# mks0601/ExAvatar_RELEASE

Hardware: AMD Instinct MI355X
Metric: train iters/sec (fwd+bwd raster) at 1024x1024 / ~150k Gaussians (higher is better)
Workload: dtype f32

## Files before the change

### exavatar_release_amd/csrc/blend.h

```cpp
#pragma once
#include "common.h"

namespace exa {

typedef float v2f __attribute__((ext_vector_type(2)));
typedef float v4f __attribute__((ext_vector_type(4)));

struct BatchLds {
    float px[BATCH], py[BATCH], ca[BATCH], cb[BATCH], cc[BATCH], op[BATCH];
    float4 col[BATCH];
};

__device__ __forceinline__ void stage_splat(BatchLds& s, int lane, const float2& r0, const float4& r1, const float4& r2) {
    s.px[lane] = r0.x; s.py[lane] = r0.y;
    s.ca[lane] = r1.x; s.cb[lane] = r1.y; s.cc[lane] = r1.z; s.op[lane] = __builtin_amdgcn_logf(r1.w);
    s.col[lane] = r2;
}

__device__ __forceinline__ bool conic_safe(float ca, float cb, float cc) {
    const float tr = ca + cc;
    return ca <= 0.0f && cc <= 0.0f && 4.0f * ca * cc - cb * cb >= 1e-5f * (tr * tr);
}

struct Alpha2 { v2f alpha, A, Ag, p2; bool vis0, vis1; };
__device__ __forceinline__ Alpha2 splat_alpha2(v2f px, v2f py, v2f ca, v2f cb, v2f cc, v2f lop, float fx, float fy, bool live) {
#pragma clang fp contract(off)
    const v2f dx = px - fx, dy = py - fy;
    const v2f t = __builtin_elementwise_fma(cb, dy, ca * dx);
    const v2f u = __builtin_elementwise_fma(cc * dy, dy, lop);
    Alpha2 r;
    r.p2 = __builtin_elementwise_fma(t, dx, u);
    r.A.x = __builtin_amdgcn_exp2f(r.p2.x);
    r.A.y = __builtin_amdgcn_exp2f(r.p2.y);
    const float a0 = fminf(ALPHA_MAX, r.A.x), a1 = fminf(ALPHA_MAX, r.A.y);
    r.vis0 = a0 >= ALPHA_MIN;
    r.vis1 = a1 >= ALPHA_MIN;
    r.alpha.x = r.vis0 ? a0 : 0.0f;
    r.alpha.y = r.vis1 ? a1 : 0.0f;
    r.Ag.x = (r.vis0 && live) ? r.A.x : 0.0f;
    r.Ag.y = (r.vis1 && live) ? r.A.y : 0.0f;
    return r;
}

struct Ops4 { v4f px, py, ca, cb, cc, op; };
__device__ __forceinline__ Ops4 load_ops4(const BatchLds& s, int k) {
    Ops4 o;
    o.px = *reinterpret_cast<const v4f*>(&s.px[k]);
    o.py = *reinterpret_cast<const v4f*>(&s.py[k]);
    o.ca = *reinterpret_cast<const v4f*>(&s.ca[k]);
    o.cb = *reinterpret_cast<const v4f*>(&s.cb[k]);
    o.cc = *reinterpret_cast<const v4f*>(&s.cc[k]);
    o.op = *reinterpret_cast<const v4f*>(&s.op[k]);
    return o;
}
struct Alpha4 { float alpha[4], Ag[4], p2[4]; unsigned long long took[4]; };
__device__ __forceinline__ Alpha4 splat_alpha4(const Ops4& o, float fx, float fy, bool live) {
    const Alpha2 lo = splat_alpha2(o.px.xy, o.py.xy, o.ca.xy, o.cb.xy, o.cc.xy, o.op.xy, fx, fy, live);
    const Alpha2 hi = splat_alpha2(o.px.zw, o.py.zw, o.ca.zw, o.cb.zw, o.cc.zw, o.op.zw, fx, fy, live);
    Alpha4 r;
    r.alpha[0] = lo.alpha.x; r.alpha[1] = lo.alpha.y; r.alpha[2] = hi.alpha.x; r.alpha[3] = hi.alpha.y;
    r.Ag[0] = lo.Ag.x; r.Ag[1] = lo.Ag.y; r.Ag[2] = hi.Ag.x; r.Ag[3] = hi.Ag.y;
    r.p2[0] = lo.p2.x; r.p2[1] = lo.p2.y; r.p2[2] = hi.p2.x; r.p2[3] = hi.p2.y;
    r.took[0] = __builtin_amdgcn_ballot_w64(lo.vis0); r.took[1] = __builtin_amdgcn_ballot_w64(lo.vis1);
    r.took[2] = __builtin_amdgcn_ballot_w64(hi.vis0); r.took[3] = __builtin_amdgcn_ballot_w64(hi.vis1);
    return r;
}
__device__ __forceinline__ void power_guard4(Alpha4& e, const Ops4& o, uint32_t unsafe4) {
    const float lop[4] = {o.op.x, o.op.y, o.op.z, o.op.w};
#pragma unroll
    for (int j = 0; j < 4; ++j) {
        if ((unsafe4 >> j) & 1u) {
            const bool neg = e.p2[j] <= lop[j];
            e.alpha[j] = neg ? e.alpha[j] : 0.0f;
            e.Ag[j] = neg ? e.Ag[j] : 0.0f;
            e.took[j] &= __builtin_amdgcn_ballot_w64(neg);
        }
    }
}

__device__ __forceinline__ void blend_group4(float& T, float& Tdead, unsigned long long live_mask, const float (&alpha)[4],
                                             float (&Tb)[4], float (&w)[4], float (&gate)[4]) {
#pragma clang fp contract(off)
    Tb[0] = T;
    w[0] = alpha[0] * Tb[0]; Tb[1] = Tb[0] - w[0];
    w[1] = alpha[1] * Tb[1]; Tb[2] = Tb[1] - w[1];
    w[2] = alpha[2] * Tb[2]; Tb[3] = Tb[2] - w[2];
    w[3] = alpha[3] * Tb[3];
    const float T4 = Tb[3] - w[3];
    if ((__builtin_amdgcn_ballot_w64(T4 < T_EPS) & live_mask) != 0ull) {
        const float after[4] = {Tb[1], Tb[2], Tb[3], T4};
        const bool dies = T4 < T_EPS && T > 0.0f;
        float Tn = T;
#pragma unroll
        for (int j = 0; j < 4; ++j) {
            const bool stop = after[j] < T_EPS;
            w[j] = stop ? 0.0f : w[j];
            gate[j] = stop ? 0.0f : gate[j];
            Tn = stop ? Tn : after[j];
        }
        Tdead = dies ? Tn : Tdead;
        T = (T4 < T_EPS) ? 0.0f : T4;
    } else {
        T = T4;
    }
}
__device__ __forceinline__ void blend_group4(float& T, float& Tdead, unsigned long long live_mask, const float (&alpha)[4],
                                             float (&Tb)[4], float (&w)[4]) {
    float none[4] = {0.f, 0.f, 0.f, 0.f};
    blend_group4(T, Tdead, live_mask, alpha, Tb, w, none);
}

}
```

### exavatar_release_amd/csrc/render_bwd.hip

```cpp
#include <stdlib.h>
#include "blend.h"

namespace exa {

constexpr int RBLOCK = 64;
template <int GC> struct XLayout;
template <> struct XLayout<16> {
    static constexpr int ROW = 36, GROUP = 16 * 36, FLOATS = 4 * 16 * 36;
    static constexpr int WK = ROW;
    __device__ static __forceinline__ int g(int lane) { return lane % 16; }
    __device__ static __forceinline__ int h(int lane) { return lane / 16; }
    __device__ static __forceinline__ int wbase(int lane) { return (lane / 16) * GROUP + 2 * (lane % 16); }
    __device__ static __forceinline__ int rbase(int lane) { return h(lane) * GROUP + g(lane) * ROW; }
    __device__ static __forceinline__ float reduce(float x) {
        x += __shfl_xor(x, 16, 64);
        x += __shfl_xor(x, 32, 64);
        return x;
    }
    __device__ static __forceinline__ void reduce9(float& a, float& b, float& c, float& d, float& e, float& f, float& g,
                                                   float& h, float& i) {
        a = reduce(a); b = reduce(b); c = reduce(c); d = reduce(d); e = reduce(e); f = reduce(f); g = reduce(g);
        h = reduce(h); i = reduce(i);
    }
};
// ... 127 lines not shown
            const int sx0 = r3.x & 0xffff, sx1 = r3.x >> 16, sy0 = r3.y & 0xffff;
            p.pslot = r3.w + (uint32_t)((sub.gsy - sy0) * (sx1 - sx0) + (sub.gsx - sx0));
            if (PREFIX && !trainable(h.id)) p.pslot = NO_SLOT;
        }
        const float* cf = a.bw.ckpt + (size_t)(b0 + (n + BATCH - 1) / BATCH) * (5 * 64) + lane;
        const float* cs = a.bw.ckpt + (size_t)slot * (5 * 64) + lane;
        if ((int)slot > b0) { p.cs0 = cs[0]; p.cs1 = cs[64]; p.cs2 = cs[128]; p.cs3 = cs[192]; p.cs4 = HAS_DEPTH ? cs[256] : 0.f; }
        p.cf0 = cf[0]; p.cf1 = cf[64]; p.cf2 = cf[128]; p.cf3 = cf[192]; p.cf4 = HAS_DEPTH ? cf[256] : 0.f;
        const int pxi = sub.ox + (lane & 7), pyi = sub.oy + (lane >> 3);
        if (pxi < a.grid.W && pyi < a.grid.H) {
            const size_t HW = (size_t)a.grid.W * a.grid.H;
            const size_t pix = (size_t)pyi * a.grid.W + pxi;
            p.gr = dL_dcolor[pix];
            p.gg = dL_dcolor[HW + pix];
            p.gb = dL_dcolor[2 * HW + pix];
            if (HAS_DEPTH && a.dL_ddepth) p.gd = a.dL_ddepth[pix];
            if (a.dL_dalpha) p.ga = a.dL_dalpha[pix];
        }
        return p;
    };

    uint32_t first_slot = wg * SPW;
    if (SPW == 1 && gridDim.y == 1) {
        const uint32_t m0 = a.tw.bwd_meta[0], m1 = a.tw.bwd_meta[1], magic = a.tw.bwd_meta[2];
        const uint32_t mapped = a.bw.bucket ? reinterpret_cast<const uint32_t*>(a.bw.bucket)[min(wg, nslots - 1u)] : 0u;
        if (magic == BWD_ORDER_MAGIC && a.bw.bucket) {
            if (wg >= m0 + m1) return;
            first_slot = mapped;
        }
    }
    BwdHdr hh[SPW];
    BwdPay pp[SPW];
#pragma unroll
    for (int i = 0; i < SPW; ++i) hh[i] = load_hdr(first_slot + i);
#pragma unroll
    for (int i = 0; i < SPW; ++i) pp[i] = load_pay(hh[i], first_slot + i);
#pragma unroll
    for (int rep = 0; rep < SPW; ++rep) {
    const BwdHdr& h0 = hh[rep];
    const BwdPay& p0 = pp[rep];
    const uint32_t slot = first_slot + rep;
    if (is_active(h0)) {
    const uint32_t bm_lo = __builtin_amdgcn_readfirstlane(h0.bm_lo), bm_hi = __builtin_amdgcn_readfirstlane(h0.bm_hi);
    const int st = (int)__builtin_amdgcn_readfirstlane(h0.st1) - 1;
    const int b0 = (int)(__builtin_amdgcn_readfirstlane(h0.begin) / BATCH);
    const int bq = (int)slot - b0;
    const int cnt = __popc(bm_lo) + __popc(bm_hi);
    const bool flagged = (((lane < 32 ? bm_lo : bm_hi) >> (lane & 31)) & 1u) != 0u;
    const int below = mask_rank(bm_lo, bm_hi);
    const int dst = flagged ? below : cnt + (lane - below);
    const SubTile sub = decode_subtile(st, a.grid);
    const int pxi = sub.ox + (lane & 7), pyi = sub.oy + (lane >> 3);
    const bool inside = pxi < a.grid.W && pyi < a.grid.H;
    const float fx = (float)pxi, fy = (float)pyi;
    const float gr = p0.gr, gg = p0.gg, gb = p0.gb, gd = p0.gd, ga = p0.ga;

    stage_splat(s_b, dst, p0.r0, p0.r1, p0.r2);
    s_pslot[dst] = p0.pslot;
    s_pg[(lane >> 4) * 17 + (lane & 15)] = make_float4(gr, gg, gb, gd);

    float T = inside ? 1.0f : 0.0f, Tdead = 1.0f;
    float sr = 0.f, sg = 0.f, sb = 0.f, sd = 0.f;
    if (bq > 0) {
        T = fmaxf(p0.cs0, 0.0f);
        sr = p0.cs1; sg = p0.cs2; sb = p0.cs3; sd = p0.cs4;
    }
    const float T_final = p0.cf0;
    const float tail = T_final * (ga - (bg[0] * gr + bg[1] * gg + bg[2] * gb));
    float R = (p0.cf1 - sr) * gr + (p0.cf2 - sg) * gg + (p0.cf3 - sb) * gb - tail;
    if (HAS_DEPTH) R = fmaf(p0.cf4 - sd, gd, R);
    wave_lds_fence();
    const unsigned long long unsafe = __builtin_amdgcn_ballot_w64(!conic_safe(s_b.ca[lane], s_b.cb[lane], s_b.cc[lane]));
    const unsigned long long need = PREFIX ? __ballot(lane < cnt && s_pslot[lane] != NO_SLOT) : ~0ull;

    const int g = XL::g(lane), h = XL::h(lane);
    float2* const xw_row = reinterpret_cast<float2*>(s_x + XL::wbase(lane));
    const float4* const xr_row = reinterpret_cast<const float4*>(s_x + XL::rbase(lane));

    for (int c0 = 0; c0 < cnt; c0 += GC) {
        if (__all(T == 0.0f)) break;
        const int cend = min(cnt, c0 + GC);
        {
            auto grad4 = [&](Alpha4& e, unsigned long long live_mask, const float4 (&col)[4], int k) {
                float Tb[4], w[4];
                blend_group4(T, Tdead, live_mask, e.alpha, Tb, w, e.Ag);
                float2* x = xw_row + (k - c0) * (XL::WK / 2);
#pragma unroll
                for (int u = 0; u < 4; ++u) {
                    const float4 c = col[u];
                    float cg = fmaf(c.z, gb, fmaf(c.y, gg, c.x * gr));
                    if (HAS_DEPTH) cg = fmaf(c.w, gd, cg);
                    R = fmaf(-cg, w[u], R);
                    const float inv = __builtin_amdgcn_rcpf(1.0f - e.alpha[u]);
                    const float dLda = fmaf(Tb[u], cg, -(R * inv));
                    x[u * (XL::WK / 2)] = make_float2(e.Ag[u] * dLda, w[u]);
                }
            };
            auto group4 = [&](const Ops4& ops, int k) {
                float4 col[4] = {s_b.col[k], s_b.col[k + 1], s_b.col[k + 2], s_b.col[k + 3]};
                if (!HAS_DEPTH) { keep_b128(col[0]); keep_b128(col[1]); keep_b128(col[2]); keep_b128(col[3]); }
                const bool live = T > 0.0f;
                const unsigned long long live_mask = __builtin_amdgcn_ballot_w64(live);
                Alpha4 e = splat_alpha4(ops, fx, fy, live);
                if ((unsafe >> k) & 0xfull) power_guard4(e, ops, (uint32_t)((unsafe >> k) & 0xfull));
                grad4(e, live_mask, col, k);
            };
            Ops4 opsA = load_ops4(s_b, c0);
            for (int k = c0; k < cend; k += 8) {
                const Ops4 opsB = load_ops4(s_b, (k + 4) & 63);
                group4(opsA, k);
                if (k + 4 >= cend) break;
                opsA = load_ops4(s_b, (k + 8) & 63);
                group4(opsB, k + 4);
            }
        }
        wave_lds_fence();
        if (!PREFIX || ((need >> c0) & ((1ull << GC) - 1ull)) != 0ull) {
            const int kk = c0 + g;
            float S0 = 0.f, Sx = 0.f, Sxx = 0.f, Sy = 0.f, Sxy = 0.f, dr = 0.f, dg = 0.f, db = 0.f, dz = 0.f;
#pragma unroll
            for (int j = 0; j < GC / 2; ++j) {
                const float4 v = xr_row[j];
#pragma unroll
                for (int t = 0; t < 2; ++t) {
                    const int q = 2 * j + t;
                    const float aG = t ? v.z : v.x, wq = t ? v.w : v.y;
                    const int pp = h * GC + q;
                    float4 pg = s_pg[(pp >> 4) * 17 + (pp & 15)];
                    if (!HAS_DEPTH) keep_b128(pg);
                    const float X = (float)((q & 7) - 4);
                    S0 += aG;
                    if ((q & 7) != 4) { Sx = fmaf(aG, X, Sx); Sxx = fmaf(aG, X * X, Sxx); }
                    if (q >> 3) {
                        Sy += aG;
                        if ((q & 7) != 4) Sxy = fmaf(aG, X, Sxy);
                    }
                    dr = fmaf(wq, pg.x, dr); dg = fmaf(wq, pg.y, dg); db = fmaf(wq, pg.z, db);
                    if (HAS_DEPTH) dz = fmaf(wq, pg.w, dz);
                }
            }
            const float u0 = s_b.px[kk] - (float)(sub.ox + 4), v0 = s_b.py[kk] - (float)(sub.oy + (GC / 8) * h);
            float mx = fmaf(u0, S0, -Sx), my = fmaf(v0, S0, -Sy);
            float mxx = fmaf(u0, mx - Sx, Sxx);
            float mxy = fmaf(v0, mx, fmaf(-u0, Sy, Sxy));
            float myy = fmaf(v0, my - Sy, Sy);
            float dop = S0;
            XL::reduce9(mx, my, mxx, mxy, myy, dop, dr, dg, db);
            if (HAS_DEPTH) dz = XL::reduce(dz);
            if (h == 0 && kk < cend) {
                const float inv_o = __builtin_amdgcn_exp2f(-s_b.op[kk]);
                const uint32_t ps = s_pslot[kk];
                if (!PREFIX || ps != NO_SLOT) {
                    char* dst = partial_at(prec, ps);
                    *reinterpret_cast<partial_v4*>(dst) = partial_v4{mx, my, mxx, mxy};
                    *reinterpret_cast<partial_v4*>(dst + 16) = partial_v4{myy, dop * inv_o, dr, dg};
                    if (PARTIAL_BYTES == 40) *reinterpret_cast<partial_v2*>(dst + 32) = partial_v2{db, dz};
                    else *reinterpret_cast<partial_v4*>(dst + 32) = partial_v4{db, dz, 0.f, 0.f};
                    if (PARTIAL_BYTES == 64) *reinterpret_cast<partial_v4*>(dst + 48) = partial_v4{0.f, 0.f, 0.f, 0.f};
                    touched[ps] = (uint8_t)1;
                }
            }
        }
        wave_lds_fence();
    }
    }
    }
}

hipError_t launch_render_bwd(const RenderBwdArgs* a, int K, hipStream_t s) {
    uint64_t slots = 0;
    bool depth = false, prefix = false;
    for (int k = 0; k < K; ++k) {
        uint64_t mine = a[k].capacity / BATCH;
        if (a[k].used_slots && a[k].used_slots < mine) mine = a[k].used_slots;
        slots = mine > slots ? mine : slots;
        depth = depth || a[k].dL_ddepth != nullptr;
        prefix = prefix || a[k].grad_first > 0;
    }
    if (slots == 0) return hipSuccess;
#ifndef EXA_BWD_GC
#define EXA_BWD_GC 8
#endif
#ifndef EXA_BWD_SPW
#define EXA_BWD_SPW 1
#endif
#ifndef EXA_BWD_WPB
#define EXA_BWD_WPB 1
#endif
#ifndef EXA_BWD_LDS_PAD
#define EXA_BWD_LDS_PAD 0
#endif
    constexpr int GC = EXA_BWD_GC, SPW = EXA_BWD_SPW, WPB = EXA_BWD_WPB;
    const Batch<RenderBwdArgs> b = make_batch(a, K);
    const dim3 grid((unsigned)((slots + SPW * WPB - 1) / (SPW * WPB)), K);
    if (prefix) {
        const dim3 g1((unsigned)((slots + WPB - 1) / WPB), K);
        if (depth) render_bwd_kernel<true, GC, 1, true, WPB><<<g1, RBLOCK * WPB, (size_t)EXA_BWD_LDS_PAD, s>>>(b);
        else render_bwd_kernel<false, GC, 1, true, WPB><<<g1, RBLOCK * WPB, (size_t)EXA_BWD_LDS_PAD, s>>>(b);
    } else if (depth) {
        render_bwd_kernel<true, GC, SPW, false, WPB><<<grid, RBLOCK * WPB, (size_t)EXA_BWD_LDS_PAD, s>>>(b);
    } else {
        render_bwd_kernel<false, GC, SPW, false, WPB><<<grid, RBLOCK * WPB, (size_t)EXA_BWD_LDS_PAD, s>>>(b);
    }
// ... 5 lines not shown
```

### exavatar_release_amd/csrc/render_fwd.hip

```cpp
#include <stdlib.h>
#include "blend.h"

namespace exa {

constexpr int RBLOCK = 64;

constexpr int SORT_TILE = 2048;
constexpr int SBLOCK = 256;

template <int E>
__device__ __forceinline__ void lds_merge_sort(const unsigned long long* gkeys, int n, uint32_t* __restrict__ sorted,
                                               unsigned long long* keys_out, unsigned long long* buf, int tid) {
    constexpr int NPAD = SBLOCK * E;
    const int lane = tid & 63;
    unsigned long long key[E];
#pragma unroll
    for (int e = 0; e < E; ++e) {
        const int i = e * SBLOCK + tid;
        key[e] = i < n ? gkeys[i] : ~0ull;
        buf[i] = key[e];
    }
    __syncthreads();
    {
        uint32_t rank[E];
// ... 389 lines not shown
        static_assert(ORDER_LDS_WORDS <= SORT_TILE, "order_slots borrows the bucket counters of the sort");
        order_slots(a.tw, a.store_ctx ? reinterpret_cast<uint32_t*>(a.bw.bucket) : nullptr, a.grid.subtiles, (int)blockIdx.x, tid,
                    s_cnt, [&](int st) { return a.tw.ranges[st]; });
        return;
    }
#ifdef EXA_PROBE_SORT
    const unsigned long long t0 = __builtin_readcyclecounter();
#endif
    if (blockIdx.x == ORDER_WGS && tid == 0 && (uint64_t)a.tw.header->num_rendered > a.capacity) a.tw.header->overflow = 1u;
    const int wg = (int)blockIdx.x - ORDER_WGS;
    if (wg >= (int)a.tw.header->active_cells * SUBS_PER_CELL) return;
    if (SPLIT && a.tw.cell_long[wg >> 6] == 0u) return;
    const int st = (int)a.tw.cell_desc[wg >> 6].x * SUBS_PER_CELL + (wg & 63);
    const uint2 range = a.tw.ranges[st];
    const int n = (int)(range.y - range.x);
    if (n == 0) return;
    unsigned long long* gkeys = a.bw.keys + range.x;
    uint32_t* sorted = a.bw.sorted + range.x;
    unsigned long long* const keys_out = KEEP ? gkeys : nullptr;
    if (n <= 64) {
        if (!SPLIT && tid < 64) wave_rank_sort64(gkeys, n, sorted, keys_out, s_buf, tid);
        return;
    }
    if (n > SORT_TILE) {
        for (int first = 0; first < n; first += 8 * SBLOCK) rank_sort_list<8>(gkeys, n, first, sorted, s_buf, tid);
        if (keys_out) {
            __threadfence_block();
            __syncthreads();
            for (int i = tid; i < n; i += SBLOCK) {
                const uint32_t id = sorted[i];
                keys_out[i] = ((unsigned long long)__float_as_uint(a.splats[id].depth) << 32) | id;
            }
        }
        return;
    }
    bool done;
    if (n <= 256) done = lds_bucket_sort<1>(gkeys, n, sorted, keys_out, s_buf, s_cnt, s_misc, tid);
    else if (n <= 512) done = lds_bucket_sort<2>(gkeys, n, sorted, keys_out, s_buf, s_cnt, s_misc, tid);
    else if (n <= 1024) done = lds_bucket_sort<4>(gkeys, n, sorted, keys_out, s_buf, s_cnt, s_misc, tid);
    else done = lds_bucket_sort<8>(gkeys, n, sorted, keys_out, s_buf, s_cnt, s_misc, tid);
    if (done) return;
    __syncthreads();
    if (n <= 256) lds_merge_sort<1>(gkeys, n, sorted, keys_out, s_buf, tid);
    else if (n <= 512) lds_merge_sort<2>(gkeys, n, sorted, keys_out, s_buf, tid);
    else if (n <= 1024) lds_merge_sort<4>(gkeys, n, sorted, keys_out, s_buf, tid);
    else lds_merge_sort<8>(gkeys, n, sorted, keys_out, s_buf, tid);
#ifdef EXA_PROBE_SORT
    __syncthreads();
    if (tid == 0) a.tw.part_cnt[st] = (uint32_t)(__builtin_readcyclecounter() - t0);
#endif
}

template <bool STORE, bool TWO>
__global__ __launch_bounds__(RBLOCK) void render_fwd_kernel(Batch<RenderFwdArgs> batch) {
    __shared__ BatchLds s_b;

    const RenderFwdArgs& a = batch.v[blockIdx.y];
    if ((int)blockIdx.x >= a.grid.subtiles) return;
    const int lane = threadIdx.x;
#ifdef EXA_PROBE_FWD
    const unsigned long long t0 = wall_clock64();
#endif
    const uint4 slot = a.tw.slots[blockIdx.x];
    const SubTile sub = decode_subtile((int)slot.z, a.grid);
    const int st = sub.st;
    if (sub.ox >= a.grid.W || sub.oy >= a.grid.H) return;
    const int pxi = sub.ox + (lane & 7), pyi = sub.oy + (lane >> 3);
    const bool inside = pxi < a.grid.W && pyi < a.grid.H;
    const float fx = (float)pxi, fy = (float)pyi;
    const uint2 range = TWO ? a.tw.ranges[slot.z] : make_uint2(slot.x, slot.y);
    const int n = (int)(range.y - range.x);
    if (TWO && n == 0 && reuse_a_pixels(a.src_color, a.src_bg, a.bg)) {
        if (inside) {
            const size_t HW = (size_t)a.grid.W * a.grid.H, pix = (size_t)pyi * a.grid.W + pxi;
            const float c0 = a.src_color[pix], c1 = a.src_color[HW + pix], c2 = a.src_color[2 * HW + pix];
            const float d = a.src_depth[pix], al = a.src_alpha[pix];
            a.out_color[pix] = c0; a.out_color[HW + pix] = c1; a.out_color[2 * HW + pix] = c2;
            a.out_depth[pix] = d; a.out_alpha[pix] = al;
        }
        if (STORE && lane == 0) a.tw.fwd_exit[st] = make_uint2(0u, 0u);
        return;
    }

    float T = inside ? 1.0f : 0.0f, Tdead = 1.0f;
    v2f Crg = {0.f, 0.f}, Cbd = {0.f, 0.f};
    const Splat* __restrict__ splats = a.splats;
    const uint32_t* __restrict__ sorted = a.bw.sorted + range.x;
    auto record = [&](uint32_t id) -> const float4* {
        if (TWO) return reinterpret_cast<const float4*>(((id & SRC_B) ? a.splats2 : splats) + (id & ~SRC_B));
        return reinterpret_cast<const float4*>(splats + id);
    };

    uint32_t id_next = 0;
    float2 r0 = make_float2(0.f, 0.f);
    float4 r1 = make_float4(0.f, 0.f, 0.f, 0.f), r2 = r1;
    if (n > 0) {
        const uint32_t id0 = lane < n ? sorted[lane] : 0u;
        if (64 + lane < n) id_next = sorted[64 + lane];
        if (lane < n) {
            const float4* rec = record(id0);
            r0 = *reinterpret_cast<const float2*>(rec); r1 = rec[1]; r2 = rec[2];
        }
    }
    float* ckpt = a.bw.ckpt + (size_t)(range.x / BATCH) * (5 * 64) + lane;
    int entered = 0;
    for (int base = 0; base < n; base += 64) {
        if (__all(T == 0.0f)) break;
        if (STORE && base > 0) {
            float* c = ckpt + (size_t)entered * (5 * 64);
            c[0] = T > 0.0f ? T : -Tdead; c[64] = Crg.x; c[128] = Crg.y; c[192] = Cbd.x; c[256] = Cbd.y;
        }
        ++entered;
        const unsigned long long unsafe = __builtin_amdgcn_ballot_w64(!conic_safe(r1.x, r1.y, r1.z));
        stage_splat(s_b, lane, r0, r1, r2);
        {
            const int jn = base + 64 + lane;
            r0 = make_float2(0.f, 0.f); r1 = make_float4(0.f, 0.f, 0.f, 0.f); r2 = r1;
            if (jn < n) {
                const float4* rec = record(id_next);
                r0 = *reinterpret_cast<const float2*>(rec); r1 = rec[1]; r2 = rec[2];
            }
            if (jn + 64 < n) id_next = sorted[jn + 64];
        }
        wave_lds_fence();
        const int cnt = min(64, n - base);
        unsigned long long blended = 0ull;
        auto blend4 = [&](const Alpha4& e, const float4& c0, const float4& c1, const float4& c2, const float4& c3, int k) -> bool {
#ifdef EXA_FWD_SKIP_VOTE
            const float amax = fmaxf(fmaxf(e.alpha[0], e.alpha[1]), fmaxf(e.alpha[2], e.alpha[3])) * T;
            if (!__any(amax > 0.0f)) return false;
#endif
            const unsigned long long live_mask = __builtin_amdgcn_ballot_w64(T > 0.0f);
            if (STORE) {
                auto vote_bit = [&](int j, uint32_t bit) -> uint32_t {
                    const unsigned long long m = e.took[j] & live_mask;
                    uint32_t r;
                    asm("s_cmp_lg_u64 %1, 0\n\ts_cselect_b32 %0, %2, 0" : "=s"(r) : "s"(m), "s"(bit) : "scc");
                    return r;
                };
                const uint32_t nib = vote_bit(0, 1u) | vote_bit(1, 2u) | vote_bit(2, 4u) | vote_bit(3, 8u);
                blended |= (unsigned long long)nib << k;
            }
            float Tb[4], w[4];
            blend_group4(T, Tdead, live_mask, e.alpha, Tb, w);
            Crg = __builtin_elementwise_fma(v2f{c0.x, c0.y}, v2f{w[0], w[0]}, Crg);
            Cbd = __builtin_elementwise_fma(v2f{c0.z, c0.w}, v2f{w[0], w[0]}, Cbd);
            Crg = __builtin_elementwise_fma(v2f{c1.x, c1.y}, v2f{w[1], w[1]}, Crg);
            Cbd = __builtin_elementwise_fma(v2f{c1.z, c1.w}, v2f{w[1], w[1]}, Cbd);
            Crg = __builtin_elementwise_fma(v2f{c2.x, c2.y}, v2f{w[2], w[2]}, Crg);
            Cbd = __builtin_elementwise_fma(v2f{c2.z, c2.w}, v2f{w[2], w[2]}, Cbd);
            Crg = __builtin_elementwise_fma(v2f{c3.x, c3.y}, v2f{w[3], w[3]}, Crg);
            Cbd = __builtin_elementwise_fma(v2f{c3.z, c3.w}, v2f{w[3], w[3]}, Cbd);
#ifdef EXA_FWD_EXIT4
            return __all(T == 0.0f);
#else
            return (k & 4) ? __all(T == 0.0f) : false;
#endif
        };
        auto group4 = [&](const Ops4& ops, int k) -> bool {
            const float4 c0 = s_b.col[k], c1 = s_b.col[k + 1], c2 = s_b.col[k + 2], c3 = s_b.col[k + 3];
            Alpha4 e = splat_alpha4(ops, fx, fy, true);
            if ((unsafe >> k) & 0xfull) power_guard4(e, ops, (uint32_t)((unsafe >> k) & 0xfull));
            return blend4(e, c0, c1, c2, c3, k);
        };
        Ops4 opsA = load_ops4(s_b, 0);
        for (int k = 0; k < cnt; k += 8) {
            const Ops4 opsB = load_ops4(s_b, (k + 4) & 63);
            if (group4(opsA, k)) break;
            if (k + 4 >= cnt) break;
            opsA = load_ops4(s_b, (k + 8) & 63);
            if (group4(opsB, k + 4)) break;
        }
        if (STORE && lane == 0) a.bw.bmask[range.x / BATCH + (uint32_t)(entered - 1)] = blended;
        wave_lds_fence();
    }

    const size_t HW = (size_t)a.grid.W * a.grid.H;
    if (inside) {
        const size_t pix = (size_t)pyi * a.grid.W + pxi;
        const float* __restrict__ bg = a.bg;
        const float Tf = T > 0.0f ? T : Tdead;
        a.out_color[pix] = Crg.x + Tf * bg[0];
        a.out_color[HW + pix] = Crg.y + Tf * bg[1];
        a.out_color[2 * HW + pix] = Cbd.x + Tf * bg[2];
        a.out_depth[pix] = Cbd.y;
        a.out_alpha[pix] = 1.0f - Tf;
    }
    if (STORE) {
        if (lane == 0) a.tw.fwd_exit[st] = make_uint2((uint32_t)n, (uint32_t)entered);
#ifdef EXA_PROBE_FWD
        if (lane == 0) {
            a.tw.part_cnt[4 * blockIdx.x] = (uint32_t)t0;
            a.tw.part_cnt[4 * blockIdx.x + 1] = (uint32_t)wall_clock64();
            const uint32_t hw = __builtin_amdgcn_s_getreg((31 << 11) | 4), xcc = __builtin_amdgcn_s_getreg((31 << 11) | 20);
            a.tw.part_cnt[4 * blockIdx.x + 2] = (hw & 0xffffu) | ((xcc & 0xfu) << 16);
        }
#endif
        if (n > 0) {
            float* c = ckpt + (size_t)((n + BATCH - 1) / BATCH) * (5 * 64);
            c[0] = T > 0.0f ? T : Tdead; c[64] = Crg.x; c[128] = Crg.y; c[192] = Cbd.x; c[256] = Cbd.y;
        }
    }
}

static int max_subtiles(const RenderFwdArgs* a, int K) {
    int n = 0;
    for (int k = 0; k < K; ++k) n = max(n, a[k].grid.subtiles);
    return n;
}

hipError_t launch_sort_subtiles(const RenderFwdArgs* a, int K, hipStream_t s) {
    const int subtiles = max_subtiles(a, K);
    if (subtiles == 0) return hipSuccess;
    const int split_at = dev_knobs().split_subtiles;
    bool keep = false;
    for (int k = 0; k < K; ++k) keep = keep || a[k].keep_sorted_keys != 0;
    const dim3 grid(subtiles + ORDER_WGS, K);
    if (subtiles >= split_at) {
        sort_short_kernel<<<dim3((subtiles + SBLOCK / 64 - 1) / (SBLOCK / 64), K), SBLOCK, 0, s>>>(make_batch(a, K));
        if (keep) sort_subtiles_kernel<true, true><<<grid, SBLOCK, 0, s>>>(make_batch(a, K));
        else sort_subtiles_kernel<true, false><<<grid, SBLOCK, 0, s>>>(make_batch(a, K));
    } else {
        if (keep) sort_subtiles_kernel<false, true><<<grid, SBLOCK, 0, s>>>(make_batch(a, K));
        else sort_subtiles_kernel<false, false><<<grid, SBLOCK, 0, s>>>(make_batch(a, K));
    }
    return hipGetLastError();
}

#ifndef EXA_FWD_LDS_PAD
#define EXA_FWD_LDS_PAD 0
#endif
hipError_t launch_render_fwd(const RenderFwdArgs* a, int K, hipStream_t s) {
    const int subtiles = max_subtiles(a, K);
    if (subtiles == 0) return hipSuccess;
    constexpr int pad = EXA_FWD_LDS_PAD;
    if (a[0].splats2) {
        if (a[0].store_ctx) render_fwd_kernel<true, true><<<dim3(subtiles, K), RBLOCK, (size_t)pad, s>>>(make_batch(a, K));
        else render_fwd_kernel<false, true><<<dim3(subtiles, K), RBLOCK, (size_t)pad, s>>>(make_batch(a, K));
    } else if (a[0].store_ctx)
        render_fwd_kernel<true, false><<<dim3(subtiles, K), RBLOCK, (size_t)pad, s>>>(make_batch(a, K));
    else
        render_fwd_kernel<false, false><<<dim3(subtiles, K), RBLOCK, (size_t)pad, s>>>(make_batch(a, K));
    return hipGetLastError();
}

}
```

### exavatar_release_amd/csrc/api.hip

```cpp
#include <stdio.h>
#include <stdlib.h>
#include <string.h>

#include "common.h"

using namespace exa;

namespace {

thread_local char g_err[512] = "";

int fail(int code, const char* what) {
    snprintf(g_err, sizeof(g_err), "exa_raster: %s", what);
    return code;
}
int fail_hip(hipError_t e, const char* where) {
    snprintf(g_err, sizeof(g_err), "exa_raster: HIP error %d (%s) in %s", (int)e, hipGetErrorString(e), where);
    return (int)e;
}

#define EXA_HIP(expr, where)                                   \
    do {                                                       \
        hipError_t e_ = (expr);                                \
        if (e_ != hipSuccess) return fail_hip(e_, where);      \
// ... 19 lines not shown
};
Timing g_t;

#define EXA_TIMED(slot, expr, where)                                        \
    do {                                                                    \
        if (g_t.enabled) EXA_HIP(hipEventRecord(g_t.ev[slot][0], st), where); \
        EXA_HIP((expr), where);                                             \
        if (g_t.enabled) {                                                  \
            EXA_HIP(hipEventRecord(g_t.ev[slot][1], st), where);            \
            g_t.used[slot] = true;                                          \
        }                                                                   \
    } while (0)

int check_settings(const ExaRasterSettings* s) {
    if (!s) return fail(EXA_RASTER_E_NULLPTR, "settings is NULL");
    if (s->image_height < 0 || s->image_width < 0) return fail(EXA_RASTER_E_INVALID, "negative image size");
    if (make_grid(s->image_width, s->image_height).cells > MAX_CELLS || s->image_width > 32768 || s->image_height > 32768)
        return fail(EXA_RASTER_E_INVALID, "image too large (more than 4096 cells of 64x64 pixels)");
    if (!s->bg || !s->viewmatrix || !s->projmatrix || !s->campos)
        return fail(EXA_RASTER_E_NULLPTR, "settings bg/viewmatrix/projmatrix/campos must be device pointers");
    if (!(s->tanfovx > 0.f) || !(s->tanfovy > 0.f)) return fail(EXA_RASTER_E_INVALID, "tanfov must be > 0");
    if (s->sh_degree < 0 || s->sh_degree > 3) return fail(EXA_RASTER_E_INVALID, "sh_degree must be 0..3");
    return 0;
}

int check_inputs(int32_t P, int32_t sh_M, const float* means3D, const float* shs, const float* colors_precomp,
                 const float* opacities, const float* scales, const float* rotations, const float* cov3D_precomp,
                 int sh_degree) {
    if (P < 0) return fail(EXA_RASTER_E_INVALID, "P < 0");
    if (P == 0) return 0;
    if (P > (1 << 26) - 4) return fail(EXA_RASTER_E_INVALID, "more than 2^26 - 4 Gaussians (32-bit byte offsets of the 64-byte splat records)");
    if (!means3D || !opacities) return fail(EXA_RASTER_E_NULLPTR, "means3D / opacities is NULL");
    if ((shs == nullptr) == (colors_precomp == nullptr))
        return fail(EXA_RASTER_E_INVALID, "provide exactly one of shs / colors_precomp");
    const bool has_sr = scales != nullptr && rotations != nullptr;
    if ((scales != nullptr) != (rotations != nullptr) || has_sr == (cov3D_precomp != nullptr))
        return fail(EXA_RASTER_E_INVALID, "provide exactly one of (scales + rotations) / cov3D_precomp");
    if (shs && sh_M < (sh_degree + 1) * (sh_degree + 1))
        return fail(EXA_RASTER_E_INVALID, "sh_M smaller than (sh_degree + 1)^2");
    return 0;
}

}

const exa::DevKnobs& exa::dev_knobs() {
    static const DevKnobs k = [] {
        DevKnobs d;
        const char* e = getenv("EXA_FOOTPRINT");
        d.footprint = !e || atoi(e) != 0;
        e = getenv("EXA_BIN_SINGLE_CELLS");
        d.single_cells = e ? atoi(e) : SINGLE_PART_CELLS;
        e = getenv("EXA_SORT_SPLIT_SUBTILES");
        d.split_subtiles = e ? atoi(e) : SPLIT_SORT_SUBTILES;
        return d;
    }();
    return k;
}

extern "C" {

int exa_raster_version(void) { return EXA_RASTER_VERSION; }

const char* exa_raster_last_error(void) { return g_err; }

int exa_raster_workspace_sizes(int32_t P, int32_t W, int32_t H, uint64_t capacity, ExaRasterWorkspaceSizes* out) {
    if (!out) return fail(EXA_RASTER_E_NULLPTR, "out is NULL");
    if (P < 0 || W < 0 || H < 0) return fail(EXA_RASTER_E_INVALID, "negative size");
    const Grid g = make_grid(W, H);
    out->geom_bytes = align256(uint64_t(P) * sizeof(Splat));
    out->tile_bytes = tile_ws_bytes(g.cells, num_chunks(P));
    out->bin_bytes = bin_ws_bytes(capacity);
    out->grad_bytes = grad_ws_bytes(capacity) + group_scratch_bytes((uint64_t)P);
    return 0;
}

}

namespace {

int check_forward_job(const ExaRasterForwardJob& j, bool stage1, bool stage2) {
    int rc = check_settings(j.settings);
    if (rc) return rc;
    if (stage1) {
        rc = check_inputs(j.P, j.sh_M, j.means3D, j.shs, j.colors_precomp, j.opacities, j.scales, j.rotations,
                          j.cov3D_precomp, j.settings->sh_degree);
        if (rc) return rc;
        if (j.P > 0 && !j.radii) return fail(EXA_RASTER_E_WORKSPACE, "workspace / radii is NULL");
    }
    if (j.P < 0) return fail(EXA_RASTER_E_INVALID, "P < 0");
    if (!j.tile_ws || (j.P > 0 && !j.geom_ws)) return fail(EXA_RASTER_E_WORKSPACE, "workspace / radii is NULL");
    if (stage2) {
        if (j.capacity > 0 && !j.bin_ws) return fail(EXA_RASTER_E_WORKSPACE, "workspace is NULL");
        if (j.capacity % BATCH) return fail(EXA_RASTER_E_INVALID, "capacity must be a multiple of 64");
        if (!j.out_color || !j.out_depth || !j.out_alpha) return fail(EXA_RASTER_E_NULLPTR, "output image is NULL");
    }
    return 0;
}

BinArgs bin_args(const ExaRasterForwardJob& j) {
    BinArgs b;
    b.P = j.P; b.chunks = num_chunks(j.P); b.merged = 0;
    b.grid = make_grid(j.settings->image_width, j.settings->image_height);
    b.splats = static_cast<Splat*>(j.geom_ws);
    b.tw = carve_tile_ws(j.tile_ws, b.grid.cells, b.chunks);
    b.bw = carve_bin_ws(j.bin_ws, j.capacity);
    b.capacity = j.capacity;
// ... 601 lines not shown
```

### exavatar_release_amd/csrc/common.h

```cpp
#pragma once
#include <hip/hip_runtime.h>
#include <stdint.h>
#include "../../include/exa_raster.h"

namespace exa {

constexpr int TILE = EXA_RASTER_TILE;
constexpr int SUB = 8;
constexpr int CELL_SUBS = 8;
constexpr int CELL = SUB * CELL_SUBS;
constexpr int SUBS_PER_CELL = CELL_SUBS * CELL_SUBS;
constexpr int BLOCK = 256;
constexpr int CHUNK = 1024;
constexpr int MAX_CELLS = 4096;
constexpr int HEADER_BYTES = 2560;

#ifndef EXA_MAX_BATCH
#define EXA_MAX_BATCH 8
#endif
constexpr int MAX_BATCH = EXA_MAX_BATCH;
template <typename T> struct Batch { T v[MAX_BATCH]; };
template <typename T>
inline Batch<T> make_batch(const T* a, int K) {
    Batch<T> b;
// ... 272 lines not shown
__host__ __device__ inline uint64_t compose_zero_bytes(uint64_t cap, uint64_t cap_b) {
    return align256((cap / BATCH + 1) * 16) + align256((cap / BATCH + 1) * 8) + align256(cap_b);
}
__host__ __device__ inline uint64_t compose_bin_bytes(uint64_t cap, uint64_t cap_b) {
    return align256(cap * 4) + compose_zero_bytes(cap, cap_b) + align256((cap / BATCH + 1) * 5 * 64 * 4);
}
__host__ __device__ inline BinWs carve_compose_ws(void* base, uint64_t cap, uint64_t cap_b) {
    BinWs b;
    char* p = static_cast<char*>(base);
    b.keys = nullptr; b.bucket = nullptr;
    b.sorted = reinterpret_cast<uint32_t*>(p); p += align256(cap * 4);
    b.owner = reinterpret_cast<uint4*>(p); p += align256((cap / BATCH + 1) * 16);
    b.bmask = reinterpret_cast<unsigned long long*>(p); p += align256((cap / BATCH + 1) * 8);
    b.touched = reinterpret_cast<uint8_t*>(p); p += align256(cap_b);
    b.ckpt = reinterpret_cast<float*>(p);
    return b;
}
hipError_t launch_render_fwd(const RenderFwdArgs* a, int K, hipStream_t s);

struct RenderBwdArgs {
    Grid grid; uint64_t capacity; int P;
    const Splat* splats; TileWs tw; BinWs bw; const float* bg;
    const float* dL_dcolor; const float* dL_ddepth; const float* dL_dalpha;
    const float* const* dL_dcolor_ind;
    uint32_t used_slots;
    PartialWs partials;
    int grad_first;
    const Splat* splats2;
    int P2;
};
hipError_t launch_render_bwd(const RenderBwdArgs* a, int K, hipStream_t s);

struct PreprocessBwdArgs {
    int P, sh_M, sh_degree;
    Grid grid;
    float tanfovx, tanfovy, focal_x, focal_y, scale_modifier;
    const float* viewmatrix; const float* projmatrix; const float* campos;
    const float* means3D; const float* shs; const float* opacities;
    const float* scales; const float* rotations; const float* cov3D_precomp;
    const int32_t* radii; const Splat* splats; PartialWs partials; const uint8_t* touched;
    uint64_t partial_bytes;
    const ExaRasterHeader* header;
    float* dL_dmeans2D; float* dL_dmeans3D; float* dL_dcolors; float* dL_dopacity;
    float* dL_dscales; float* dL_drotations; float* dL_dsh; float* dL_dcov3D;
    float* dens_accum; float* dens_cnt; float* dens_rmax;
    int grad_first;
    int accumulate;
    float* group_scratch;
};
hipError_t launch_preprocess_bwd(const PreprocessBwdArgs* a, int K, int sum_shared, int dens_shared, hipStream_t s);

constexpr int SINGLE_PART_CELLS = 1024;
constexpr int SPLIT_SORT_SUBTILES = 65536;
struct DevKnobs {
    bool footprint;
    int single_cells;
    int split_subtiles;
};
const DevKnobs& dev_knobs();
hipError_t launch_ssim_fwd(int N, int H, int W, const float* img1, const float* img2, float* map, float* dm_dmu1,
                           float* dm_dE11, float* dm_dE12, hipStream_t s);
hipError_t launch_ssim_bwd(int N, int H, int W, const float* img1, const float* img2, const float* dL_dmap,
                           const float* dm_dmu1, const float* dm_dE11, const float* dm_dE12, float* dL_dimg1,
                           hipStream_t s);
hipError_t launch_photo_loss(int B, int C, int H, int W, const int* crop, const float* x, const float* y, const float* l1w,
                             const float* smask, float w_l1, float w_ssim, float* maps, float* partials, float* dL_dx,
                             int stage, hipStream_t s);
hipError_t launch_l1(int B, int C, int H, int W, const int* crop, const float* x, const float* y, const float* mask,
                     const float* bg, const float* g, float* out, int backward, hipStream_t s);
hipError_t launch_densify_stats(int P, const float* g2d, const int32_t* radii, float* accum, float* cnt, float* rmax,
                                hipStream_t s);

}
```

Before: 7669.

## Precompute per-splat quadratic coefficients relative to subtile centre for alpha evaluation

Each splat's Gaussian exponent is re-expanded once per batch as a quadratic in the pixel offset from the 8x8 subtile centre, storing linear and constant terms (cu, cv, cw) in LDS instead of position and log-opacity. The per-pixel alpha evaluation then becomes a few packed FMAs with op_sel broadcasting of the lane offset, which removes the per-pair subtraction work. Log-opacity and position are no longer kept in LDS: the power guard reads them through readlane, and the backward pass fetches them with ds_permute/bpermute. The cost is extra per-splat setup, some cross-lane traffic, and possible rounding differences from the re-centred expansion.

```diff
diff --git a/exavatar_release_amd/csrc/blend.h b/exavatar_release_amd/csrc/blend.h
--- a/exavatar_release_amd/csrc/blend.h
+++ b/exavatar_release_amd/csrc/blend.h
@@ -6,15 +6,43 @@
 typedef float v2f __attribute__((ext_vector_type(2)));
 typedef float v4f __attribute__((ext_vector_type(4)));
 
+typedef v2f LanePos;
+__device__ __forceinline__ LanePos lane_pos(int lane) { return v2f{(float)(lane & 7) - 3.5f, (float)(lane >> 3) - 3.5f}; }
+__device__ __forceinline__ v2f pk_fma_lo(v2f a, v2f c, v2f b) {
+    v2f r;
+    asm("v_pk_fma_f32 %0, %1, %2, %3 op_sel_hi:[1,0,1]" : "=v"(r) : "v"(a), "v"(c), "v"(b));
+    return r;
+}
+__device__ __forceinline__ v2f pk_fma_hi(v2f a, v2f c, v2f b) {
+    v2f r;
+    asm("v_pk_fma_f32 %0, %1, %2, %3 op_sel:[0,1,0]" : "=v"(r) : "v"(a), "v"(c), "v"(b));
+    return r;
+}
+__device__ __forceinline__ float2 subtile_centre(int ox, int oy) { return make_float2((float)ox + 3.5f, (float)oy + 3.5f); }
+
+struct Quad { float u, v, w; };
+__device__ __forceinline__ Quad splat_quad(float px, float py, float ca, float cb, float cc, float lop, float2 c) {
+#pragma clang fp contract(off)
+    const float mx = px - c.x, my = py - c.y;
+    Quad q;
+    q.u = -__builtin_fmaf(2.0f * ca, mx, cb * my);
+    q.v = -__builtin_fmaf(2.0f * cc, my, cb * mx);
+    q.w = __builtin_fmaf(__builtin_fmaf(cb, my, ca * mx), mx, __builtin_fmaf(cc * my, my, lop));
+    return q;
+}
+
 struct BatchLds {
-    float px[BATCH], py[BATCH], ca[BATCH], cb[BATCH], cc[BATCH], op[BATCH];
+    float ca[BATCH], cb[BATCH], cc[BATCH], cu[BATCH], cv[BATCH], cw[BATCH];
     float4 col[BATCH];
 };
 
-__device__ __forceinline__ void stage_splat(BatchLds& s, int lane, const float2& r0, const float4& r1, const float4& r2) {
-    s.px[lane] = r0.x; s.py[lane] = r0.y;
-    s.ca[lane] = r1.x; s.cb[lane] = r1.y; s.cc[lane] = r1.z; s.op[lane] = __builtin_amdgcn_logf(r1.w);
-    s.col[lane] = r2;
+__device__ __forceinline__ float stage_splat(BatchLds& s, int idx, const float2& r0, const float4& r1, const float4& r2, float2 c) {
+    const float lop = __builtin_amdgcn_logf(r1.w);
+    const Quad q = splat_quad(r0.x, r0.y, r1.x, r1.y, r1.z, lop, c);
+    s.ca[idx] = r1.x; s.cb[idx] = r1.y; s.cc[idx] = r1.z;
+    s.cu[idx] = q.u; s.cv[idx] = q.v; s.cw[idx] = q.w;
+    s.col[idx] = r2;
+    return lop;
 }
 
 __device__ __forceinline__ bool conic_safe(float ca, float cb, float cc) {
@@ -23,13 +51,12 @@
 }
 
 struct Alpha2 { v2f alpha, A, Ag, p2; bool vis0, vis1; };
-__device__ __forceinline__ Alpha2 splat_alpha2(v2f px, v2f py, v2f ca, v2f cb, v2f cc, v2f lop, float fx, float fy, bool live) {
+__device__ __forceinline__ Alpha2 splat_alpha2(v2f ca, v2f cb, v2f cc, v2f cu, v2f cv, v2f cw, const LanePos& q, bool live) {
 #pragma clang fp contract(off)
-    const v2f dx = px - fx, dy = py - fy;
-    const v2f t = __builtin_elementwise_fma(cb, dy, ca * dx);
-    const v2f u = __builtin_elementwise_fma(cc * dy, dy, lop);
+    const v2f a = pk_fma_lo(ca, q, pk_fma_hi(cb, q, cu));
+    const v2f b = pk_fma_hi(cc, q, cv);
     Alpha2 r;
-    r.p2 = __builtin_elementwise_fma(t, dx, u);
+    r.p2 = pk_fma_hi(b, q, pk_fma_lo(a, q, cw));
     r.A.x = __builtin_amdgcn_exp2f(r.p2.x);
     r.A.y = __builtin_amdgcn_exp2f(r.p2.y);
     const float a0 = fminf(ALPHA_MAX, r.A.x), a1 = fminf(ALPHA_MAX, r.A.y);
@@ -42,21 +69,21 @@
     return r;
 }
 
-struct Ops4 { v4f px, py, ca, cb, cc, op; };
+struct Ops4 { v4f ca, cb, cc, cu, cv, cw; };
 __device__ __forceinline__ Ops4 load_ops4(const BatchLds& s, int k) {
     Ops4 o;
-    o.px = *reinterpret_cast<const v4f*>(&s.px[k]);
-    o.py = *reinterpret_cast<const v4f*>(&s.py[k]);
     o.ca = *reinterpret_cast<const v4f*>(&s.ca[k]);
     o.cb = *reinterpret_cast<const v4f*>(&s.cb[k]);
     o.cc = *reinterpret_cast<const v4f*>(&s.cc[k]);
-    o.op = *reinterpret_cast<const v4f*>(&s.op[k]);
+    o.cu = *reinterpret_cast<const v4f*>(&s.cu[k]);
+    o.cv = *reinterpret_cast<const v4f*>(&s.cv[k]);
+    o.cw = *reinterpret_cast<const v4f*>(&s.cw[k]);
     return o;
 }
 struct Alpha4 { float alpha[4], Ag[4], p2[4]; unsigned long long took[4]; };
-__device__ __forceinline__ Alpha4 splat_alpha4(const Ops4& o, float fx, float fy, bool live) {
-    const Alpha2 lo = splat_alpha2(o.px.xy, o.py.xy, o.ca.xy, o.cb.xy, o.cc.xy, o.op.xy, fx, fy, live);
-    const Alpha2 hi = splat_alpha2(o.px.zw, o.py.zw, o.ca.zw, o.cb.zw, o.cc.zw, o.op.zw, fx, fy, live);
+__device__ __forceinline__ Alpha4 splat_alpha4(const Ops4& o, const LanePos& q, bool live) {
+    const Alpha2 lo = splat_alpha2(o.ca.xy, o.cb.xy, o.cc.xy, o.cu.xy, o.cv.xy, o.cw.xy, q, live);
+    const Alpha2 hi = splat_alpha2(o.ca.zw, o.cb.zw, o.cc.zw, o.cu.zw, o.cv.zw, o.cw.zw, q, live);
     Alpha4 r;
     r.alpha[0] = lo.alpha.x; r.alpha[1] = lo.alpha.y; r.alpha[2] = hi.alpha.x; r.alpha[3] = hi.alpha.y;
     r.Ag[0] = lo.Ag.x; r.Ag[1] = lo.Ag.y; r.Ag[2] = hi.Ag.x; r.Ag[3] = hi.Ag.y;
@@ -65,12 +92,12 @@
     r.took[2] = __builtin_amdgcn_ballot_w64(hi.vis0); r.took[3] = __builtin_amdgcn_ballot_w64(hi.vis1);
     return r;
 }
-__device__ __forceinline__ void power_guard4(Alpha4& e, const Ops4& o, uint32_t unsafe4) {
-    const float lop[4] = {o.op.x, o.op.y, o.op.z, o.op.w};
+__device__ __forceinline__ void power_guard4(Alpha4& e, float lop_lane, int k, uint32_t unsafe4) {
 #pragma unroll
     for (int j = 0; j < 4; ++j) {
         if ((unsafe4 >> j) & 1u) {
-            const bool neg = e.p2[j] <= lop[j];
+            const float lop = __builtin_bit_cast(float, __builtin_amdgcn_readlane(__builtin_bit_cast(int, lop_lane), k + j));
+            const bool neg = e.p2[j] <= lop;
             e.alpha[j] = neg ? e.alpha[j] : 0.0f;
             e.Ag[j] = neg ? e.Ag[j] : 0.0f;
             e.took[j] &= __builtin_amdgcn_ballot_w64(neg);
diff --git a/exavatar_release_amd/csrc/render_bwd.hip b/exavatar_release_amd/csrc/render_bwd.hip
--- a/exavatar_release_amd/csrc/render_bwd.hip
+++ b/exavatar_release_amd/csrc/render_bwd.hip
@@ -203,10 +203,14 @@
     const SubTile sub = decode_subtile(st, a.grid);
     const int pxi = sub.ox + (lane & 7), pyi = sub.oy + (lane >> 3);
     const bool inside = pxi < a.grid.W && pyi < a.grid.H;
-    const float fx = (float)pxi, fy = (float)pyi;
+    const LanePos q = lane_pos(lane);
     const float gr = p0.gr, gg = p0.gg, gb = p0.gb, gd = p0.gd, ga = p0.ga;
 
-    stage_splat(s_b, dst, p0.r0, p0.r1, p0.r2);
+    const float lop = stage_splat(s_b, dst, p0.r0, p0.r1, p0.r2, subtile_centre(sub.ox, sub.oy));
+    auto to_entry = [&](float v) {
+        return __builtin_bit_cast(float, __builtin_amdgcn_ds_permute(dst << 2, __builtin_bit_cast(int, v)));
+    };
+    const float e_px = to_entry(p0.r0.x), e_py = to_entry(p0.r0.y), e_lop = to_entry(lop);
     s_pslot[dst] = p0.pslot;
     s_pg[(lane >> 4) * 17 + (lane & 15)] = make_float4(gr, gg, gb, gd);
 
@@ -252,8 +256,8 @@
                 if (!HAS_DEPTH) { keep_b128(col[0]); keep_b128(col[1]); keep_b128(col[2]); keep_b128(col[3]); }
                 const bool live = T > 0.0f;
                 const unsigned long long live_mask = __builtin_amdgcn_ballot_w64(live);
-                Alpha4 e = splat_alpha4(ops, fx, fy, live);
-                if ((unsafe >> k) & 0xfull) power_guard4(e, ops, (uint32_t)((unsafe >> k) & 0xfull));
+                Alpha4 e = splat_alpha4(ops, q, live);
+                if ((unsafe >> k) & 0xfull) power_guard4(e, e_lop, k, (uint32_t)((unsafe >> k) & 0xfull));
                 grad4(e, live_mask, col, k);
             };
             Ops4 opsA = load_ops4(s_b, c0);
@@ -290,7 +294,11 @@
                     if (HAS_DEPTH) dz = fmaf(wq, pg.w, dz);
                 }
             }
-            const float u0 = s_b.px[kk] - (float)(sub.ox + 4), v0 = s_b.py[kk] - (float)(sub.oy + (GC / 8) * h);
+            auto of_entry = [&](float v) {
+                return __builtin_bit_cast(float, __builtin_amdgcn_ds_bpermute(kk << 2, __builtin_bit_cast(int, v)));
+            };
+            const float k_px = of_entry(e_px), k_py = of_entry(e_py), k_lop = of_entry(e_lop);
+            const float u0 = k_px - (float)(sub.ox + 4), v0 = k_py - (float)(sub.oy + (GC / 8) * h);
             float mx = fmaf(u0, S0, -Sx), my = fmaf(v0, S0, -Sy);
             float mxx = fmaf(u0, mx - Sx, Sxx);
             float mxy = fmaf(v0, mx, fmaf(-u0, Sy, Sxy));
@@ -299,7 +307,7 @@
             XL::reduce9(mx, my, mxx, mxy, myy, dop, dr, dg, db);
             if (HAS_DEPTH) dz = XL::reduce(dz);
             if (h == 0 && kk < cend) {
-                const float inv_o = __builtin_amdgcn_exp2f(-s_b.op[kk]);
+                const float inv_o = __builtin_amdgcn_exp2f(-k_lop);
                 const uint32_t ps = s_pslot[kk];
                 if (!PREFIX || ps != NO_SLOT) {
                     char* dst = partial_at(prec, ps);
diff --git a/exavatar_release_amd/csrc/render_fwd.hip b/exavatar_release_amd/csrc/render_fwd.hip
--- a/exavatar_release_amd/csrc/render_fwd.hip
+++ b/exavatar_release_amd/csrc/render_fwd.hip
@@ -480,7 +480,8 @@
     if (sub.ox >= a.grid.W || sub.oy >= a.grid.H) return;
     const int pxi = sub.ox + (lane & 7), pyi = sub.oy + (lane >> 3);
     const bool inside = pxi < a.grid.W && pyi < a.grid.H;
-    const float fx = (float)pxi, fy = (float)pyi;
+    const LanePos q = lane_pos(lane);
+    const float2 centre = subtile_centre(sub.ox, sub.oy);
     const uint2 range = TWO ? a.tw.ranges[slot.z] : make_uint2(slot.x, slot.y);
     const int n = (int)(range.y - range.x);
     if (TWO && n == 0 && reuse_a_pixels(a.src_color, a.src_bg, a.bg)) {
@@ -525,7 +526,7 @@
         }
         ++entered;
         const unsigned long long unsafe = __builtin_amdgcn_ballot_w64(!conic_safe(r1.x, r1.y, r1.z));
-        stage_splat(s_b, lane, r0, r1, r2);
+        const float lop = stage_splat(s_b, lane, r0, r1, r2, centre);
         {
             const int jn = base + 64 + lane;
             r0 = make_float2(0.f, 0.f); r1 = make_float4(0.f, 0.f, 0.f, 0.f); r2 = r1;
@@ -572,8 +573,8 @@
         };
         auto group4 = [&](const Ops4& ops, int k) -> bool {
             const float4 c0 = s_b.col[k], c1 = s_b.col[k + 1], c2 = s_b.col[k + 2], c3 = s_b.col[k + 3];
-            Alpha4 e = splat_alpha4(ops, fx, fy, true);
-            if ((unsafe >> k) & 0xfull) power_guard4(e, ops, (uint32_t)((unsafe >> k) & 0xfull));
+            Alpha4 e = splat_alpha4(ops, q, true);
+            if ((unsafe >> k) & 0xfull) power_guard4(e, lop, k, (uint32_t)((unsafe >> k) & 0xfull));
             return blend4(e, c0, c1, c2, c3, k);
         };
         Ops4 opsA = load_ops4(s_b, 0);
```

Measured after the change: 7698 (median of 6 runs). No clear change (+0.4%).

## Compact live pixels across lanes in forward blend when few remain

Applied to the files above, without the earlier changes.

When at most a set number of pixels in a 64-lane wave are still unsaturated (T>0), the forward render gathers their state into groups of four lanes with ds_permute/bpermute. Each lane in a group then evaluates one splat of a four-splat batch, and DPP broadcasts share the alphas inside the group. Afterwards the results are scattered back to the owning lanes. The aim is to replace mostly idle lanes with useful splat evaluations once most pixels have terminated, at the cost of permute overhead, extra code size and register pressure.

```diff
diff --git a/exavatar_release_amd/csrc/api.hip b/exavatar_release_amd/csrc/api.hip
--- a/exavatar_release_amd/csrc/api.hip
+++ b/exavatar_release_amd/csrc/api.hip
@@ -95,6 +95,8 @@
         d.single_cells = e ? atoi(e) : SINGLE_PART_CELLS;
         e = getenv("EXA_SORT_SPLIT_SUBTILES");
         d.split_subtiles = e ? atoi(e) : SPLIT_SORT_SUBTILES;
+        e = getenv("EXA_PIX_COMPACT");
+        d.pix_compact = e ? atoi(e) : EXA_PIX_COMPACT_DEFAULT;
         return d;
     }();
     return k;
diff --git a/exavatar_release_amd/csrc/blend.h b/exavatar_release_amd/csrc/blend.h
--- a/exavatar_release_amd/csrc/blend.h
+++ b/exavatar_release_amd/csrc/blend.h
@@ -39,6 +39,20 @@
     r.alpha.y = r.vis1 ? a1 : 0.0f;
     r.Ag.x = (r.vis0 && live) ? r.A.x : 0.0f;
     r.Ag.y = (r.vis1 && live) ? r.A.y : 0.0f;
+    return r;
+}
+
+struct Alpha1 { float alpha, p2; bool vis; };
+__device__ __forceinline__ Alpha1 splat_alpha1(float px, float py, float ca, float cb, float cc, float lop, float fx, float fy) {
+#pragma clang fp contract(off)
+    const float dx = px - fx, dy = py - fy;
+    const float t = __builtin_fmaf(cb, dy, ca * dx);
+    const float u = __builtin_fmaf(cc * dy, dy, lop);
+    Alpha1 r;
+    r.p2 = __builtin_fmaf(t, dx, u);
+    const float a = fminf(ALPHA_MAX, __builtin_amdgcn_exp2f(r.p2));
+    r.vis = a >= ALPHA_MIN;
+    r.alpha = r.vis ? a : 0.0f;
     return r;
 }
 
diff --git a/exavatar_release_amd/csrc/common.h b/exavatar_release_amd/csrc/common.h
--- a/exavatar_release_amd/csrc/common.h
+++ b/exavatar_release_amd/csrc/common.h
@@ -348,10 +348,14 @@
 
 constexpr int SINGLE_PART_CELLS = 1024;
 constexpr int SPLIT_SORT_SUBTILES = 65536;
+#ifndef EXA_PIX_COMPACT_DEFAULT
+#define EXA_PIX_COMPACT_DEFAULT 16
+#endif
 struct DevKnobs {
     bool footprint;
     int single_cells;
     int split_subtiles;
+    int pix_compact;
 };
 const DevKnobs& dev_knobs();
 hipError_t launch_ssim_fwd(int N, int H, int W, const float* img1, const float* img2, float* map, float* dm_dmu1,
diff --git a/exavatar_release_amd/csrc/render_fwd.hip b/exavatar_release_amd/csrc/render_fwd.hip
--- a/exavatar_release_amd/csrc/render_fwd.hip
+++ b/exavatar_release_amd/csrc/render_fwd.hip
@@ -465,7 +465,7 @@
 }
 
 template <bool STORE, bool TWO>
-__global__ __launch_bounds__(RBLOCK) void render_fwd_kernel(Batch<RenderFwdArgs> batch) {
+__global__ __launch_bounds__(RBLOCK) void render_fwd_kernel(Batch<RenderFwdArgs> batch, int compact) {
     __shared__ BatchLds s_b;
 
     const RenderFwdArgs& a = batch.v[blockIdx.y];
@@ -576,13 +576,93 @@
             if ((unsafe >> k) & 0xfull) power_guard4(e, ops, (uint32_t)((unsafe >> k) & 0xfull));
             return blend4(e, c0, c1, c2, c3, k);
         };
-        Ops4 opsA = load_ops4(s_b, 0);
-        for (int k = 0; k < cnt; k += 8) {
-            const Ops4 opsB = load_ops4(s_b, (k + 4) & 63);
-            if (group4(opsA, k)) break;
-            if (k + 4 >= cnt) break;
-            opsA = load_ops4(s_b, (k + 8) & 63);
-            if (group4(opsB, k + 4)) break;
+        const unsigned long long live0 = __builtin_amdgcn_ballot_w64(T > 0.0f);
+        const int nlive = __popcll(live0);
+        auto walk_compact = [&]() {
+            constexpr unsigned long long M0 = 0x1111111111111111ull;
+            auto pull = [](float v, int from) { return __int_as_float(__builtin_amdgcn_ds_bpermute(from << 2, __float_as_int(v))); };
+            int l = lane;
+            asm volatile("" : "+v"(l));
+            const int rank = (int)__builtin_amdgcn_mbcnt_hi((uint32_t)(live0 >> 32), __builtin_amdgcn_mbcnt_lo((uint32_t)live0, 0u));
+            const bool was_live = (live0 >> l) & 1ull;
+            const int owner = __builtin_amdgcn_ds_permute((was_live ? rank : nlive + l - rank) << 2, l);
+            const int src = __builtin_amdgcn_ds_bpermute((l >> 2) << 2, owner);
+            float cT = pull(T, src), cTd = pull(Tdead, src);
+            v2f cRg = {pull(Crg.x, src), pull(Crg.y, src)}, cBd = {pull(Cbd.x, src), pull(Cbd.y, src)};
+            const float cfx = (float)(sub.ox + (src & 7)), cfy = (float)(sub.oy + (src >> 3));
+            const int jl = l & 3;
+            struct COps { float px, py, ca, cb, cc, op; };
+            auto load = [&](int k) {
+                const int e = k + jl;
+                return COps{s_b.px[e], s_b.py[e], s_b.ca[e], s_b.cb[e], s_b.cc[e], s_b.op[e]};
+            };
+            auto cgroup = [&](const COps& o, int k) -> bool {
+                float alpha[4];
+                unsigned long long took[4];
+                const uint32_t unsafe4 = (uint32_t)((unsafe >> k) & 0xfull);
+                {
+                    Alpha1 r = splat_alpha1(o.px, o.py, o.ca, o.cb, o.cc, o.op, cfx, cfy);
+                    unsigned long long m = __builtin_amdgcn_ballot_w64(r.vis);
+                    if (unsafe4) {
+                        const bool keep = !((unsafe4 >> jl) & 1u) || r.p2 <= o.op;
+                        r.alpha = keep ? r.alpha : 0.0f;
+                        m &= __builtin_amdgcn_ballot_w64(keep);
+                    }
+#pragma unroll
+                    for (int j = 0; j < 4; ++j) took[j] = m & (M0 << j);
+                    alpha[0] = __int_as_float(__builtin_amdgcn_mov_dpp(__float_as_int(r.alpha), 0x00, 0xf, 0xf, false));
+                    alpha[1] = __int_as_float(__builtin_amdgcn_mov_dpp(__float_as_int(r.alpha), 0x55, 0xf, 0xf, false));
+                    alpha[2] = __int_as_float(__builtin_amdgcn_mov_dpp(__float_as_int(r.alpha), 0xAA, 0xf, 0xf, false));
+                    alpha[3] = __int_as_float(__builtin_amdgcn_mov_dpp(__float_as_int(r.alpha), 0xFF, 0xf, 0xf, false));
+                }
+                const unsigned long long live_mask = __builtin_amdgcn_ballot_w64(cT > 0.0f);
+                if (STORE) {
+                    auto vote_bit = [&](int j, uint32_t bit) -> uint32_t {
+                        const unsigned long long m = took[j] & live_mask;
+                        uint32_t r;
+                        asm("s_cmp_lg_u64 %1, 0\n\ts_cselect_b32 %0, %2, 0" : "=s"(r) : "s"(m), "s"(bit) : "scc");
+                        return r;
+                    };
+                    const uint32_t nib = vote_bit(0, 1u) | vote_bit(1, 2u) | vote_bit(2, 4u) | vote_bit(3, 8u);
+                    blended |= (unsigned long long)nib << k;
+                }
+                const float4 c0 = s_b.col[k], c1 = s_b.col[k + 1], c2 = s_b.col[k + 2], c3 = s_b.col[k + 3];
+                float Tb[4], w[4];
+                blend_group4(cT, cTd, live_mask, alpha, Tb, w);
+                cRg = __builtin_elementwise_fma(v2f{c0.x, c0.y}, v2f{w[0], w[0]}, cRg);
+                cBd = __builtin_elementwise_fma(v2f{c0.z, c0.w}, v2f{w[0], w[0]}, cBd);
+                cRg = __builtin_elementwise_fma(v2f{c1.x, c1.y}, v2f{w[1], w[1]}, cRg);
+                cBd = __builtin_elementwise_fma(v2f{c1.z, c1.w}, v2f{w[1], w[1]}, cBd);
+                cRg = __builtin_elementwise_fma(v2f{c2.x, c2.y}, v2f{w[2], w[2]}, cRg);
+                cBd = __builtin_elementwise_fma(v2f{c2.z, c2.w}, v2f{w[2], w[2]}, cBd);
+                cRg = __builtin_elementwise_fma(v2f{c3.x, c3.y}, v2f{w[3], w[3]}, cRg);
+                cBd = __builtin_elementwise_fma(v2f{c3.z, c3.w}, v2f{w[3], w[3]}, cBd);
+                return (k & 4) ? __all(cT == 0.0f) : false;
+            };
+            COps oA = load(0);
+            for (int k = 0; k < cnt; k += 8) {
+                const COps oB = load((k + 4) & 63);
+                if (cgroup(oA, k)) break;
+                if (k + 4 >= cnt) break;
+                oA = load((k + 8) & 63);
+                if (cgroup(oB, k + 4)) break;
+            }
+            const int from = rank << 2;
+            const float nT = pull(cT, from), nTd = pull(cTd, from);
+            const v2f nRg = {pull(cRg.x, from), pull(cRg.y, from)}, nBd = {pull(cBd.x, from), pull(cBd.y, from)};
+            if (was_live) { T = nT; Tdead = nTd; Crg = nRg; Cbd = nBd; }
+        };
+        if (nlive <= compact) {
+            walk_compact();
+        } else {
+            Ops4 opsA = load_ops4(s_b, 0);
+            for (int k = 0; k < cnt; k += 8) {
+                const Ops4 opsB = load_ops4(s_b, (k + 4) & 63);
+                if (group4(opsA, k)) break;
+                if (k + 4 >= cnt) break;
+                opsA = load_ops4(s_b, (k + 8) & 63);
+                if (group4(opsB, k + 4)) break;
+            }
         }
         if (STORE && lane == 0) a.bw.bmask[range.x / BATCH + (uint32_t)(entered - 1)] = blended;
         wave_lds_fence();
@@ -647,13 +727,14 @@
     const int subtiles = max_subtiles(a, K);
     if (subtiles == 0) return hipSuccess;
     constexpr int pad = EXA_FWD_LDS_PAD;
+    const int compact = min(16, max(0, dev_knobs().pix_compact));
     if (a[0].splats2) {
-        if (a[0].store_ctx) render_fwd_kernel<true, true><<<dim3(subtiles, K), RBLOCK, (size_t)pad, s>>>(make_batch(a, K));
-        else render_fwd_kernel<false, true><<<dim3(subtiles, K), RBLOCK, (size_t)pad, s>>>(make_batch(a, K));
+        if (a[0].store_ctx) render_fwd_kernel<true, true><<<dim3(subtiles, K), RBLOCK, (size_t)pad, s>>>(make_batch(a, K), compact);
+        else render_fwd_kernel<false, true><<<dim3(subtiles, K), RBLOCK, (size_t)pad, s>>>(make_batch(a, K), compact);
     } else if (a[0].store_ctx)
-        render_fwd_kernel<true, false><<<dim3(subtiles, K), RBLOCK, (size_t)pad, s>>>(make_batch(a, K));
+        render_fwd_kernel<true, false><<<dim3(subtiles, K), RBLOCK, (size_t)pad, s>>>(make_batch(a, K), compact);
     else
-        render_fwd_kernel<false, false><<<dim3(subtiles, K), RBLOCK, (size_t)pad, s>>>(make_batch(a, K));
+        render_fwd_kernel<false, false><<<dim3(subtiles, K), RBLOCK, (size_t)pad, s>>>(make_batch(a, K), compact);
     return hipGetLastError();
 }
 
```

After: 7655 before, 7644 after (median of 3 runs). About the same (-0.1%).
